# uncbiag/OAI_analysis_2

Hardware: NVIDIA B200
Metric: knee volumes/sec (seg+ICON reg+warp) (higher is better)
Workload: dtype fp16 operands / fp32 accumulate (tcgen05 kind::f16), the full-resolution decoder layers read fp16 hi+lo activations (dc2: skip input only; dc1); fp32 registration; fp64 warp coordinates

## Files before the change

### oai_analysis_2_b200/csrc/api_conv.cu

```cuda
#include "../../include/oai_b200.h"
#include "api_common.h"
#include "conv_api.h"
#include "conv_igemm.cuh"

#include <cuda_bf16.h>
#include <cuda_fp16.h>

#include <cstring>
#include <vector>

namespace oai {

cudaError_t conv_igemm_launch(const ConvIgemmParams& p, const CUtensorMap& tm0, const CUtensorMap& tm1, int num_sms,
                              cudaStream_t stream);
cudaError_t conv_overflow_count(unsigned int* count, bool reset, cudaStream_t stream);

namespace {

constexpr int kFlagForcePerTap = 1;
constexpr int kFlagBaseOffFormula = 2;
constexpr int kFlagForceKd1 = 4;
constexpr int kFlagNoFastPath = 8;
constexpr int kFlagWideN = 16;
constexpr int kFlagWideRows = 32;
// ... 20 lines not shown

int build_chunks(const ConvSpec& s, Plan* pl) {
  int n = 0;
  const int cs[2] = {s.c0, s.c1};
  for (int src = 0; src < 2; ++src) {
    const int c = cs[src];
    if (c == 0) continue;
    const bool spl = split_src(s.terms, src);
    const int wide = spl ? 2 * c : c;
    for (int j = 0; j * 64 < wide; ++j) {
      OAI_REQUIRE(n < kMaxChunks, "conv plan: more than %d K chunks", kMaxChunks);
      pl->chunks[n++] = Chunk{src, j * 64, s.terms == 3 ? 1 : 0, spl ? 1 : 0};
    }
    if (s.terms == 3)
      for (int j = 0; j * 64 < c; ++j) {
        OAI_REQUIRE(n < kMaxChunks, "conv plan: more than %d K chunks", kMaxChunks);
        pl->chunks[n++] = Chunk{src, j * 64, 2, 0};
      }
  }
  pl->nch = n;
  return 0;
}

int make_plan(const ConvSpec& s, Plan* pl, int d_cnt = 0) {
  const int D = s.D, H = s.H, W = s.W, c0 = s.c0, c1 = s.c1, cout = s.cout, pointwise = s.kind, flags = s.flags;
  OAI_REQUIRE(D > 0 && H > 0 && W > 0 && c0 > 0 && c1 >= 0 && cout > 0, "conv plan: bad dims");
  OAI_REQUIRE(c0 % 8 == 0 && c1 % 8 == 0, "conv plan: channel counts must be multiples of 8 (got %d,%d)", c0, c1);
  OAI_REQUIRE(s.terms >= 1 && s.terms <= 5,
              "conv plan: terms=%d (1 = 16-bit, 2 = split activations, 3 = split both, 4 / 5 = split the second / first "
              "source's activations only)", s.terms);
  OAI_REQUIRE((!split_src(s.terms, 0) || s.split0) && (!split_src(s.terms, 1) || c1 == 0 || s.split1),
              "conv plan: terms=%d needs the split sources stored as [hi | lo] planes", s.terms);
  OAI_REQUIRE(s.terms < 4 || c1 > 0, "conv plan: terms=%d is for two-source layers", s.terms);
  OAI_REQUIRE((!s.split0 || c0 % 32 == 0) && (!s.split1 || c1 % 64 == 0) && (c1 == 0 || c0 % 64 == 0),
              "conv plan: split / concatenated sources need 64-channel multiples (got %d,%d)", c0, c1);
  pl->TW = W < 128 ? W : 128;
  OAI_REQUIRE(128 % pl->TW == 0 && W % pl->TW == 0, "conv plan: W=%d must divide or be a multiple of 128", W);
  pl->TH = 128 / pl->TW;
  OAI_REQUIRE(H % pl->TH == 0, "conv plan: H=%d not a multiple of the %d-row M tile", H, pl->TH);
  const int ntile = (!pointwise && cout > 128 && !(flags & kFlagWideN)) ? 128 : 256;
  pl->nhalf = (cout + ntile - 1) / ntile;
  OAI_REQUIRE(cout % pl->nhalf == 0, "conv plan: cout=%d not divisible into %d N splits", cout, pl->nhalf);
  pl->cph = cout / pl->nhalf;
  OAI_REQUIRE(pl->cph % 32 == 0, "conv plan: cout per split (%d) must be a multiple of 32", pl->cph);
  OAI_REQUIRE(cout <= 512, "conv plan: cout=%d exceeds the 512-float bias staging area", cout);
  if (d_cnt <= 0) d_cnt = D;
  int R = 512 / pl->cph < 8 ? 512 / pl->cph : 8;
  if (R > d_cnt) R = d_cnt;
  pl->R = R;
  pl->Rd = R;
  pl->up_groups = 1;
  pl->pingpong = 0;
  if (build_chunks(s, pl)) return 1;
  const int c0v = split_src(s.terms, 0) ? 2 * c0 : c0;
  pl->k16 = (c1 == 0 && c0v <= 32) ? (c0v <= 16 ? 1 : 2) : 4;
  pl->row_bytes = (c1 == 0 && c0v == 32 && !(flags & kFlagWideRows)) ? 64 : 128;
  const int rb = pl->row_bytes;
  const int nch = pl->nch;
  if (pointwise == 2) {
    pl->mode = kModeUp2;
    pl->kd_per_block = 1;
    pl->R = 512 / pl->cph < 8 ? 512 / pl->cph : 8;
    if (pl->R >= 2 && !(flags & (kFlagNoFastPath | kFlagBaseOffFormula | kFlagNoPingPong))) {
      pl->R /= 2;
      pl->pingpong = 1;
    }
    pl->Rd = 1;
    pl->up_groups = 8 / pl->R;
    pl->wblock_bytes = pl->R * pl->cph * rb;
    pl->nblk = nch;
    pl->n_wbuf = 2;
  } else if (pointwise) {
    pl->mode = kModePointwise;
    pl->kd_per_block = 1;
    pl->wblock_bytes = pl->cph * rb;
    pl->nblk = nch;
    pl->n_wbuf = 3;
  } else if (pl->TW == 128 && pl->cph <= 64 && !(flags & kFlagForcePerTap)) {
    pl->mode = kModeRowShared;
    pl->kd_per_block = 3;
    pl->wblock_bytes = 9 * pl->cph * rb;
    pl->nblk = nch * 3;
    pl->n_wbuf = 2;
  } else {
    pl->mode = kModePerTap;
    pl->kd_per_block = (pl->cph <= 128 && !(flags & kFlagForceKd1)) ? 3 : 1;
    pl->wblock_bytes = pl->kd_per_block * pl->cph * rb;
    pl->nblk = nch * (pl->kd_per_block == 3 ? 9 : 27);
    pl->n_wbuf = pl->kd_per_block == 3 ? 2 : 3;
  }
  pl->nkh = 1;
  if (pl->mode == kModeRowShared && rb == 64 && nch == 1 &&
      !(flags & (kFlagOneKhRow | kFlagNoFastPath | kFlagBaseOffFormula))) {
    pl->nkh = 3;
    pl->n_wbuf = 1;
  }
  pl->astage_bytes = (pl->mode == kModeRowShared ? 130 : 128) * rb * pl->nkh;
  pl->astage_stride = (pl->astage_bytes + 1023u) & ~1023u;
  const size_t wstride = (static_cast<size_t>(pl->wblock_bytes) * pl->nkh + 1023u) & ~size_t(1023);
  pl->stationary = 0;
  if (pl->nkh == 3) pl->stationary = 1;
  if (pl->mode == kModeUp2 && pl->pingpong && pl->nblk <= 4 && pl->nblk * wstride + 4 * pl->astage_stride <= kSmemBudget) {
    pl->stationary = 1;
    pl->n_wbuf = pl->nblk;
  }
  const size_t left = kSmemBudget - pl->n_wbuf * wstride;
  int ns = static_cast<int>(left / pl->astage_stride);
  if (ns > 8) ns = 8;
  OAI_REQUIRE(ns >= 2, "conv plan: shared memory budget leaves %d A stages", ns);
  pl->n_astage = ns;
  return 0;
}

size_t plan_wpack_bytes(const Plan& pl) {
  return static_cast<size_t>(pl.nhalf) * pl.up_groups * pl.nblk * pl.wblock_bytes;
}

typedef CUresult (*EncodeTiledFn)(CUtensorMap*, CUtensorMapDataType, cuuint32_t, void*, const cuuint64_t*,
                                  const cuuint64_t*, const cuuint32_t*, const cuuint32_t*, CUtensorMapInterleave,
                                  CUtensorMapSwizzle, CUtensorMapL2promotion, CUtensorMapFloatOOBfill);
// ... 96 lines not shown
  if (s.terms == 3) { q[1].resize(nw); q[2].resize(nw); }
  for (size_t f = 0; f < static_cast<size_t>(cout) * cin; ++f) {
    double carry = 0.0;
    for (int t = 0; t < ktaps; ++t) {
      const double v = static_cast<double>(w[f * ktaps + t]) + (s.kind == 2 ? 0.0 : carry);
      const uint16_t h = to16(static_cast<float>(v), fmt);
      q[0][f * ktaps + t] = h;
      carry = v - static_cast<double>(from16(h, fmt));
      if (s.terms == 3) {
        const float wf = w[f * ktaps + t];
        const uint16_t hi = to16(wf, fmt);
        q[1][f * ktaps + t] = hi;
        q[2][f * ktaps + t] = to16(wf - from16(hi, fmt), fmt);
      }
    }
  }
  const int cs[2] = {s.c0, s.c1};
  const int ngroups = pl.up_groups;
  for (int nh = 0; nh < pl.nhalf; ++nh)
    for (int tg = 0; tg < ngroups; ++tg)
      for (int b = 0; b < pl.nblk; ++b) {
        uint8_t* blk = out + ((static_cast<size_t>(nh) * ngroups + tg) * pl.nblk + b) * pl.wblock_bytes;
        int c, kh = 0, kw0 = 0, nkw = 1, kdlo = 0, nkd = 1;
        if (pl.mode == kModeRowShared) {
          c = b / 3; kh = b % 3; nkw = 3; nkd = 3;
        } else if (pl.mode == kModePerTap && pl.kd_per_block == 3) {
          c = b / 9; const int r = b % 9; kh = r / 3; kw0 = r % 3; nkd = 3;
        } else if (pl.mode == kModePerTap) {
          c = b / 27; const int r = b % 27; kh = r / 9; kw0 = (r / 3) % 3; kdlo = r % 3;
        } else {
          c = b;
        }
        const Chunk& ck = pl.chunks[c];
        const int csrc = cs[ck.src], cbase = ck.src == 0 ? 0 : s.c0;
        const std::vector<uint16_t>& qq = q[ck.wsel];
        const int nstack = pl.mode == kModeUp2 ? pl.R : nkd;
        for (int kwi = 0; kwi < nkw; ++kwi)
          for (int ti = 0; ti < nstack; ++ti) {
            int tap;
            if (pl.mode == kModeUp2) tap = tg * pl.R + ti;
            else if (s.kind == 1) tap = 0;
            else tap = ((kdlo + nkd - 1 - ti) * 3 + kh) * 3 + kw0 + kwi;
            for (int co = 0; co < pl.cph; ++co) {
              const int r = (kwi * nstack + ti) * pl.cph + co;
              const uint16_t* wrow = qq.data() + (static_cast<size_t>(nh * pl.cph + co) * cin) * ktaps;
              for (int j = 0; j < 64 && j * 2 < pl.row_bytes; ++j) {
                const int v = ck.cc + j;
                if (v >= (ck.dup ? 2 * csrc : csrc)) break;
                const int ci = cbase + (ck.dup ? v % csrc : v);
                const uint16_t h = wrow[static_cast<size_t>(ci) * ktaps + tap];
                memcpy(blk + swz_off(r, j, pl.row_bytes), &h, 2);
              }
            }
          }
      }
  return 0;
}

int conv_run(const ConvSpec& s, const ConvLaunch& a, cudaStream_t st) {
  const int D = s.D, H = s.H, W = s.W, c0 = s.c0, c1 = s.c1, cout = s.cout;
  int d_lo = 0, d_cnt = D, h_lo = 0, h_cnt = H;
  if (a.region) {
    d_lo = a.region[0]; d_cnt = a.region[1]; h_lo = a.region[2]; h_cnt = a.region[3];
    OAI_REQUIRE(d_lo >= 0 && d_cnt >= 1 && d_lo + d_cnt <= D && h_lo >= 0 && h_cnt >= 1 && h_lo + h_cnt <= H,
                "conv: region [%d,+%d)x[%d,+%d) outside %dx%d", d_lo, d_cnt, h_lo, h_cnt, D, H);
  }
  Plan pl;
  if (make_plan(s, &pl, d_cnt)) return 1;
  const int hp_lo = h_lo / pl.TH;
  const int hp_cnt = (h_lo + h_cnt + pl.TH - 1) / pl.TH - hp_lo;
  const HeadFuse* head = a.head;
  OAI_REQUIRE(a.src0 && a.wpack && a.bias, "conv: null pointer");
  OAI_REQUIRE(!head || (pl.cph == 64 && pl.nhalf == 1), "conv head: the fused head needs a 64-channel layer");
  OAI_REQUIRE((c1 == 0) == (a.src1 == nullptr), "conv: src1/c1 mismatch");
  const size_t need = plan_wpack_bytes(pl);
  OAI_REQUIRE(a.wpack_bytes == need, "conv: packed weights are %zu bytes, geometry needs %zu", a.wpack_bytes, need);
  OAI_REQUIRE(a.obase % 16 == 0 && a.osN % 16 == 0 && a.osD % 16 == 0 && a.osH % 16 == 0 && a.osW % 16 == 0 &&
                  a.out_lo_off % 16 == 0 && (head || (reinterpret_cast<uintptr_t>(a.out) & 31) == 0),
              "conv: output base and strides must keep 32-byte alignment");
  OAI_REQUIRE(!(head && a.out_split), "conv head: the fused head writes class maps, not a split activation");

  ConvIgemmParams p;
  memset(&p, 0, sizeof(p));
  p.NT = a.NT; p.D = D; p.H = H; p.W = W;
  p.TW = pl.TW; p.TH = pl.TH; p.R = pl.R;
  p.cout = pl.cph; p.nhalf = pl.nhalf;
  p.nchunks = pl.nch; p.k16_steps = pl.k16; p.row_bytes = pl.row_bytes;
  for (int c = 0; c < pl.nch; ++c) {
    p.chunk_src[c] = static_cast<uint8_t>(pl.chunks[c].src);
    p.chunk_cc[c] = static_cast<uint16_t>(pl.chunks[c].cc);
  }
  p.mode = pl.mode; p.kd_per_block = pl.kd_per_block; p.nblk = pl.nblk / pl.nkh;
  p.wblock_bytes = pl.wblock_bytes * pl.nkh; p.n_wbuf = pl.n_wbuf; p.n_astage = pl.n_astage;
  p.nkh = pl.nkh;
  p.acc_pingpong = pl.pingpong;
  p.w_stationary = pl.stationary;
  p.astage_bytes = pl.astage_bytes; p.astage_stride = pl.astage_stride;
  p.ab_format = s.fmt; p.relu = a.relu;
  p.base_off_mode = (s.flags & kFlagBaseOffFormula) ? 1 : 0;
  p.no_fast_path = (s.flags & kFlagNoFastPath) ? 1 : 0;
  p.wpack = static_cast<const uint8_t*>(a.wpack);
  p.bias = a.bias;
  p.out = a.out;
  p.obase = a.obase; p.osN = a.osN; p.osD = a.osD; p.osH = a.osH; p.osW = a.osW;
  p.out_split = a.out_split; p.out_lo_off = a.out_lo_off;
  p.d_lo = d_lo; p.d_cnt = d_cnt; p.hp_lo = hp_lo; p.hp_cnt = hp_cnt;
  p.Rd = pl.Rd; p.up_groups = pl.up_groups;
  p.nunits = a.NT * ((d_cnt + pl.Rd - 1) / pl.Rd) * (hp_cnt * (W / pl.TW)) * pl.up_groups * pl.nhalf;
  if (pl.mode == kModeUp2) {
    const long long vox = a.osW / 2;
    for (int t = 0; t < 8; ++t)
      p.tap_off[t] = ((static_cast<long long>(t >> 2) * 2 * H + ((t >> 1) & 1)) * 2 * W + (t & 1)) * vox;
  }
  if (head) p.head = *head;

  OAI_REQUIRE(pl.mode != kModeUp2 || (c1 == 0 && !head), "conv: up2 mode takes one source and no fused head");
  const int bw = pl.mode == kModeRowShared ? 130 : pl.TW;
  const int bh = pl.TH * pl.nkh;
  CUtensorMap tm0, tm1;
  if (make_act_tmap(&tm0, a.src0, s.split0 ? 2 * c0 : c0, W, H, D, a.NT, bw, bh, s.fmt, pl.row_bytes)) return 1;
  if (a.src1) {
    if (make_act_tmap(&tm1, a.src1, s.split1 ? 2 * c1 : c1, W, H, D, a.NT, bw, bh, s.fmt)) return 1;
  } else {
    tm1 = tm0;
  }
  ProfEntry* pe = nullptr;
  if (g_prof_on) {
    if (g_prof_used == g_prof.size()) {
      ProfEntry ne;
      if (cudaEventCreate(&ne.a) != cudaSuccess || cudaEventCreate(&ne.b) != cudaSuccess)
        return fail("conv profile: cannot create events");
      g_prof.push_back(ne);
    }
    pe = &g_prof[g_prof_used++];
    const double taps = s.kind == 0 ? 27.0 : (s.kind == 1 ? 1.0 : 8.0);
    pe->flops = 2.0 * a.NT * D * H * W * static_cast<double>(cout) * (c0 + c1) * taps;
    pe->exec_flops = 2.0 * a.NT * static_cast<double>(d_cnt) * hp_cnt * pl.TH * W * static_cast<double>(cout) * taps *
                     (static_cast<double>(pl.nch) * pl.k16 * 16);
    prof_record(pe->a, st);
  }
  cudaError_t e = conv_igemm_launch(p, tm0, tm1, num_sms(), st);
  if (pe) prof_record(pe->b, st);
  g_launches.fetch_add(1, std::memory_order_relaxed);
  return check_cuda(e, "conv_igemm launch");
}

}

using namespace oai;

namespace {
ConvSpec spec_of(int D, int H, int W, int c0, int c1, int cout, int pointwise, int ab_format, int flags) {
  ConvSpec s;
  s.D = D; s.H = H; s.W = W; s.c0 = c0; s.c1 = c1; s.split0 = 0; s.split1 = 0; s.cout = cout; s.kind = pointwise;
  s.terms = 1; s.fmt = ab_format; s.flags = flags;
  return s;
}
}

extern "C" int oai_conv3d_igemm_plan(int D, int H, int W, int c0, int c1, int cout, int pointwise, int flags,
// ... 169 lines not shown
```

### oai_analysis_2_b200/csrc/conv_api.h

```cpp
#pragma once
#include <cstddef>
#include <cuda_runtime.h>

#include "conv_igemm.cuh"

namespace oai {

struct ConvSpec {
  int D, H, W;
  int c0, c1;
  int split0, split1;
  int cout;
  int kind;
  int terms;
  int fmt;
  int flags;
};

struct ConvLaunch {
  const void* src0;
  const void* src1;
  int NT;
  const void* wpack;
  size_t wpack_bytes;
  const float* bias;
  int relu;
  void* out;
  long long obase, osN, osD, osH, osW;
  int out_split;
  long long out_lo_off;
  const int* region;
  const HeadFuse* head;
};

size_t conv_wpack_bytes(const ConvSpec& s);
int conv_pack_weights(const ConvSpec& s, const float* w, void* dst, size_t dst_bytes);
int conv_run(const ConvSpec& s, const ConvLaunch& a, cudaStream_t st);

inline HeadFuse make_head_fuse(int ncls, const float* head_w, const float* head_b, float* out, const int* vol_dims,
                               const int* geom, int tile0, const int* crop_zyx, int out_mode) {
  HeadFuse hd;
  hd.enabled = 1; hd.ncls = ncls; hd.out_mode = out_mode; hd.w = head_w; hd.b = head_b; hd.out = out;
  hd.VD = vol_dims[0]; hd.VH = vol_dims[1]; hd.VW = vol_dims[2];
  hd.ed = geom[3]; hd.eh = geom[4]; hd.ew = geom[5];
  hd.od = geom[6]; hd.oh = geom[7]; hd.ow = geom[8];
  hd.gh = geom[10]; hd.gw = geom[11]; hd.tile0 = tile0;
  hd.cz = crop_zyx[0]; hd.cy = crop_zyx[1]; hd.cx = crop_zyx[2];
  return hd;
}

}
```

### oai_analysis_2_b200/csrc/conv_igemm.cu

```cuda
#include "conv_igemm.cuh"
#include "ptx.cuh"

#include <cuda_bf16.h>
#include <cuda_fp16.h>

namespace oai {

namespace {

constexpr int kThreads = 384;
constexpr int kEpiGroups = 2;
constexpr int kTmemCols = 512;

__device__ unsigned int g_fp16_overflow = 0;

struct BlockInfo {
  int c, kh, kw, kdlo, nkd;
  int ns;
};

__device__ __forceinline__ BlockInfo decode_block(const ConvIgemmParams& p, int b) {
  BlockInfo bi;
  if (p.mode == kModeRowShared) {
    bi.c = p.nkh == 3 ? b : b / 3;
    bi.kh = p.nkh == 3 ? 0 : b % 3;
    bi.kw = 0;
    bi.kdlo = 0;
    bi.nkd = 3;
  } else if (p.mode == kModePerTap) {
    if (p.kd_per_block == 3) {
      bi.c = b / 9;
      const int r = b % 9;
      bi.kh = r / 3;
      bi.kw = r % 3;
      bi.kdlo = 0;
      bi.nkd = 3;
    } else {
      bi.c = b / 27;
      const int r = b % 27;
      bi.kh = r / 9;
      bi.kw = (r / 3) % 3;
      bi.kdlo = r % 3;
      bi.nkd = 1;
    }
  } else {
    bi.c = b;
    bi.kh = 1;
    bi.kw = 1;
    bi.kdlo = 1;
    bi.nkd = 1;
  }
  bi.ns = (p.mode == kModeUp2) ? p.R : bi.nkd;
  return bi;
}

struct UnitInfo {
  int n, d0, h0, w0, nh;
  int tg;
  int rd;
  int ra;
};

__device__ __forceinline__ UnitInfo decode_unit(const ConvIgemmParams& p, int u) {
  UnitInfo ui;
  const int npw = p.W / p.TW;
  const int np = npw * p.hp_cnt, ndg = (p.d_cnt + p.Rd - 1) / p.Rd;
  if (p.w_stationary) {
    const int per_key = np * ndg * p.NT;
    const int key = u / per_key;
    u -= key * per_key;
    ui.tg = key % p.up_groups;
    ui.nh = key / p.up_groups;
  } else {
    ui.nh = u % p.nhalf;
    u /= p.nhalf;
    ui.tg = u % p.up_groups;
    u /= p.up_groups;
  }
  const int patch = u % np;
  u /= np;
  ui.d0 = p.d_lo + (u % ndg) * p.Rd;
  ui.n = u / ndg;
  ui.h0 = (p.hp_lo + patch / npw) * p.TH;
  ui.w0 = (patch % npw) * p.TW;
  ui.rd = min(p.Rd, p.d_lo + p.d_cnt - ui.d0);
  ui.ra = (p.mode == kModeUp2) ? p.R : ui.rd;
  return ui;
}

template <int FMT>
__device__ __forceinline__ uint32_t pack2(float a, float b) {
  if (FMT == 0) {
    __half2 h = __floats2half2_rn(a, b);
    return *reinterpret_cast<uint32_t*>(&h);
  }
  __nv_bfloat162 h = __floats2bfloat162_rn(a, b);
  return *reinterpret_cast<uint32_t*>(&h);
}

__device__ __forceinline__ void st_global_256(void* p, const uint32_t* v) {
  asm volatile("st.global.v8.b32 [%0], {%1,%2,%3,%4,%5,%6,%7,%8};" ::"l"(p), "r"(v[0]), "r"(v[1]), "r"(v[2]), "r"(v[3]),
               "r"(v[4]), "r"(v[5]), "r"(v[6]), "r"(v[7])
               : "memory");
}

template <int FMT>
__device__ __forceinline__ uint32_t pack2_residual(float a, float b, uint32_t hi) {
// ... 107 lines not shown
    const int ag = acc0 + g0;
    const int keep = min(max(f0 - ag, 0), ng);
    const uint32_t bl = b_lo + static_cast<uint32_t>(g0) * c.tap16;
    if (keep > 0)
      umma_f16_ss_lohi(tmem_base + static_cast<uint32_t>(ag) * c.cout, a_lo, bl, c.desc_hi32,
                       c.idesc_1 + static_cast<uint32_t>(keep - 1) * c.idesc_step, 1u);
    if (keep < ng)
      umma_f16_ss_lohi(tmem_base + static_cast<uint32_t>(ag + keep) * c.cout, a_lo,
                       bl + static_cast<uint32_t>(keep) * c.tap16, c.desc_hi32,
                       c.idesc_1 + static_cast<uint32_t>(ng - keep - 1) * c.idesc_step, 0u);
  }
}

template <int NKW, int K16N, int PER, int NKH>
__device__ __forceinline__ void mma_issuer_fast(const ConvIgemmParams& p, const uint32_t tmem_base0, uint8_t* abuf,
                                                uint8_t* wbuf, const uint32_t wstride, uint64_t* full_a,
                                                uint64_t* empty_a, uint64_t* full_w, uint64_t* empty_w,
                                                uint64_t* acc_full0, uint64_t* acc_empty0) {
  const int mode = p.mode, R_acc = p.R, nblk = p.nblk, nst = p.n_astage, nwb = p.n_wbuf, Dm1 = p.D - 1;
  const uint32_t rowb = static_cast<uint32_t>(p.row_bytes), sbo = 8u * rowb, lay = rowb == 128u ? 2u : 4u;
  IssueConsts c;
  c.cout = static_cast<uint32_t>(p.cout);
  c.tap16 = (c.cout * rowb) >> 4;
  c.kw_step = rowb >> 4;
  c.desc_hi32 = (sbo >> 4) | (1u << 14) | (lay << 29);
  c.idesc_1 = umma_idesc_f16(128, c.cout, p.ab_format);
  c.idesc_step = (c.cout >> 3) << 17;
  const uint32_t a_lo0 = ((smem_u32(abuf) & 0x3FFFF) >> 4) | (1u << 16), a_step = p.astage_stride >> 4;
  const uint32_t w_lo0 = ((smem_u32(wbuf) & 0x3FFFF) >> 4) | (1u << 16), w_step = wstride >> 4;
  const bool up2 = mode == kModeUp2;
  const bool one_kd = mode == kModePointwise || up2;
  const bool kd_cycle = mode == kModePerTap && p.kd_per_block == 1;
  const int ns = up2 ? R_acc : ((one_kd || kd_cycle) ? 1 : 3);
  const int a_inc = up2 ? 0 : 1;
  c.b_kw = static_cast<uint32_t>(ns) * c.tap16;
  c.kh_a = (130u * rowb) >> 4;
  c.kh_b = 3u * c.b_kw;
  const bool stationary = p.w_stationary != 0;
  int prev_key = -1;
  const bool leader = elect_one();
  int stage = 0, wb = 0;
  uint32_t aphase = 0, wphase = 0;
  uint32_t ub0 = 0, ub1 = 0;
  uint32_t a_lo = a_lo0;
  int half = 0;
  for (int u = blockIdx.x; u < p.nunits; u += gridDim.x) {
    const UnitInfo ui = decode_unit(p, u);
// ... 62 lines not shown
      }
      if (release && leader) umma_commit(&empty_w[wb]);
      if (++wb == nwb) {
        wb = 0;
        if (reload) wphase ^= 1u;
      }
    }
    if (leader && signaled != all_acc) {
      for (int a = 0; a < ra; ++a)
        if (!((signaled >> a) & 1u)) umma_commit(&acc_full[a]);
    }
    if (this_half) ub1 = use_bits ^ all_acc;
    else ub0 = use_bits ^ all_acc;
  }
  __syncwarp();
}

__device__ __forceinline__ void mma_issuer_general(const ConvIgemmParams& p, const uint32_t tmem_base, uint8_t* abuf,
                                                   uint8_t* wbuf, const uint32_t wstride, uint64_t* full_a,
                                                   uint64_t* empty_a, uint64_t* full_w, uint64_t* empty_w,
                                                   uint64_t* acc_full, uint64_t* acc_empty) {
  const int mode = p.mode, R_acc = p.R, cout = p.cout, nblk = p.nblk, nst = p.n_astage, nwb = p.n_wbuf, Dm1 = p.D - 1,
            kpb = p.kd_per_block;
  const int nkw = (mode == kModeRowShared) ? 3 : 1;
  const int k16n = p.k16_steps;
  const uint32_t rowb = static_cast<uint32_t>(p.row_bytes), sbo = 8u * rowb, lay = rowb == 128u ? 2u : 4u;
  const uint32_t cout128 = static_cast<uint32_t>(cout) * rowb;
  const bool up2 = mode == kModeUp2;
  const bool leader = elect_one();
  int stage = 0, wb = 0;
  uint32_t aphase = 0, wphase = 0, use_bits = 0;
  for (int u = blockIdx.x; u < p.nunits; u += gridDim.x) {
    const UnitInfo ui = decode_unit(p, u);
    const int d0 = ui.d0, ra = ui.ra, rd = ui.rd;
    const uint32_t all_acc = (1u << ra) - 1u;
    uint32_t touched = 0, signaled = 0;
    int kd_it = 0;
    for (int b = 0; b < nblk; ++b) {
      int kdlo = 0, nkd = 3;
      if (mode == kModePointwise || up2) { kdlo = 1; nkd = 1; }
      else if (mode == kModePerTap && kpb == 1) { kdlo = kd_it; nkd = 1; kd_it = kd_it == 2 ? 0 : kd_it + 1; }
      const int ns = up2 ? R_acc : nkd;
      const int kdhi = kdlo + nkd - 1;
      const int dlo = max(0, d0 + kdlo - 1);
      const int dhi = min(Dm1, d0 + rd - 1 + kdhi - 1);
      const bool last_blk = b == nblk - 1;
      mbar_wait(&full_w[wb], wphase, 300 + wb);
      int a_first = up2 ? 0 : dlo - kdhi + 1 - d0;
      for (int dp = dlo; dp <= dhi; ++dp, a_first += (up2 ? 0 : 1)) {
        mbar_wait(&full_a[stage], aphase, 400 + stage);
        tc_fence_after();
        const int acc0 = max(a_first, 0);
        const int ti_lo = acc0 - a_first;
        const int nt = min(ns - 1, ra - 1 - a_first) - ti_lo + 1;
        const uint32_t a_base = smem_u32(abuf + static_cast<size_t>(stage) * p.astage_stride);
        const uint32_t w_base = smem_u32(wbuf + static_cast<size_t>(wb) * wstride);
        const int ti_hi = ti_lo + nt - 1;
        for (int kw = 0; kw < nkw; ++kw) {
          int ti = ti_lo;
          while (ti <= ti_hi) {
            const int a0 = a_first + ti;
            const uint32_t f = (touched >> a0) & 1u;
            int len = 1;
            while (ti + len <= ti_hi && ((touched >> (a0 + len)) & 1u) == f && (len + 1) * cout <= 256) ++len;
            if (!f) {
              for (int j = 0; j < len; ++j)
                mbar_wait(&acc_empty[a0 + j], ((use_bits >> (a0 + j)) & 1u) ^ 1u, 500 + a0 + j);
              tc_fence_after();
            }
            const uint32_t idesc = umma_idesc_f16(128, static_cast<uint32_t>(len * cout), p.ab_format);
            const uint32_t a_addr = a_base + static_cast<uint32_t>(kw) * rowb;
            const uint32_t b_addr = w_base + static_cast<uint32_t>(kw * ns + ti) * cout128;
            const uint32_t boff = p.base_off_mode ? ((a_addr >> 7) & 7u) : 0u;
            const uint32_t d_addr = tmem_base + static_cast<uint32_t>(a0 * cout);
            if (leader) {
              for (int k16 = 0; k16 < k16n; ++k16) {
                const uint64_t adesc = umma_desc_kmajor(a_addr + k16 * 32, sbo, boff, lay);
                const uint64_t bdesc = umma_desc_kmajor(b_addr + k16 * 32, sbo, 0, lay);
                umma_f16_ss(d_addr, adesc, bdesc, idesc, (f | (k16 > 0)) ? 1u : 0u);
              }
            }
            touched |= ((1u << len) - 1u) << a0;
            ti += len;
          }
        }
        const bool publish = last_blk && a_first >= 0 && a_first < ra;
        if (leader) {
          umma_commit(&empty_a[stage]);
          if (publish) umma_commit(&acc_full[a_first]);
        }
        if (publish) signaled |= 1u << a_first;
        if (++stage == nst) {
          stage = 0;
          aphase ^= 1u;
// ... 98 lines not shown
    if (lane == 0) {
      int wb = 0, prev_key = -1;
      uint32_t phase = 0;
      for (int u = blockIdx.x; u < p.nunits; u += gridDim.x) {
        const UnitInfo ui = decode_unit(p, u);
        const uint8_t* src = p.wpack + static_cast<size_t>(ui.nh * p.up_groups + ui.tg) * p.nblk * p.wblock_bytes;
        const int key = ui.nh * p.up_groups + ui.tg;
        if (p.w_stationary && key == prev_key) continue;
        prev_key = key;
        for (int b = 0; b < p.nblk; ++b) {
          mbar_wait(&empty_w[wb], phase ^ 1u, 200 + wb);
          mbar_arrive_expect_tx(&full_w[wb], p.wblock_bytes);
          bulk_load(wbuf + static_cast<size_t>(wb) * wstride, src + static_cast<size_t>(b) * p.wblock_bytes,
                    p.wblock_bytes, &full_w[wb]);
          if (++wb == p.n_wbuf) {
            wb = 0;
            phase ^= 1u;
          }
        }
      }
    }
  } else if (warp == 2) {
    const bool general = p.base_off_mode || p.no_fast_path;
    const int nkw_rt = (p.mode == kModeRowShared) ? 3 : 1;
    const int per_rt = max(1, 256 / p.cout);
#define OAI_ISSUE(NKW, K16N, PER) \
  mma_issuer_fast<NKW, K16N, PER, 1>(p, tmem_base, abuf, wbuf, wstride, full_a, empty_a, full_w, empty_w, acc_full, acc_empty)
#define OAI_ISSUE_GENERAL() \
  mma_issuer_general(p, tmem_base, abuf, wbuf, wstride, full_a, empty_a, full_w, empty_w, acc_full, acc_empty)
    if (general) OAI_ISSUE_GENERAL();
    else if (nkw_rt == 3 && p.k16_steps == 4 && per_rt == 4) OAI_ISSUE(3, 4, 4);
    else if (nkw_rt == 3 && p.k16_steps == 2 && per_rt == 4 && p.nkh == 3)
      mma_issuer_fast<3, 2, 4, 3>(p, tmem_base, abuf, wbuf, wstride, full_a, empty_a, full_w, empty_w, acc_full, acc_empty);
    else if (nkw_rt == 3 && p.k16_steps == 2 && per_rt == 4) OAI_ISSUE(3, 2, 4);
    else if (nkw_rt == 1 && p.k16_steps == 4 && per_rt == 4) OAI_ISSUE(1, 4, 4);
    else if (nkw_rt == 1 && p.k16_steps == 4 && per_rt == 2) OAI_ISSUE(1, 4, 2);
    else if (nkw_rt == 1 && p.k16_steps == 4 && per_rt == 1) OAI_ISSUE(1, 4, 1);
    else OAI_ISSUE_GENERAL();
#undef OAI_ISSUE_GENERAL
#undef OAI_ISSUE
  } else if (warp >= 4) {
    const int q = warp & 3;
    const int eg = (warp - 4) >> 2;
    const int epi_variant = (p.ab_format ? 4 : 0) + (p.out_split ? 2 : 0) + (p.relu ? 1 : 0);
    const uint32_t s_bias_addr = smem_u32(s_bias), s_head_addr = smem_u32(s_head);
    const int m = q * 32 + lane;
    const int th = m / p.TW, tw = m % p.TW;
// ... 139 lines not shown
```

### oai_analysis_2_b200/csrc/conv_igemm.cuh

```cuda
#pragma once
#include <cstdint>
#include <cuda.h>
#include <cuda_runtime.h>

namespace oai {

constexpr int kMaxChunks = 48;

enum ConvMode : int {
  kModeRowShared = 0,
  kModePerTap = 1,
  kModePointwise = 2,
  kModeUp2 = 3,
};

struct HeadFuse {
  int enabled;
  int ncls, out_mode;
  const float* w;
  const float* b;
  float* out;
  int VD, VH, VW;
  int ed, eh, ew, od, oh, ow, gh, gw, tile0;
  int cz, cy, cx;
};

struct ConvIgemmParams {
  int NT, D, H, W;
  int TW, TH;
  int R;
  int Rd;
  int up_groups;
  long long tap_off[8];
  int d_lo, d_cnt;
  int hp_lo, hp_cnt;
  int cout;
  int nhalf;
  int nchunks;
  uint16_t chunk_cc[kMaxChunks];
  uint8_t chunk_src[kMaxChunks];
  int k16_steps;
  int row_bytes;
  int mode;
  int kd_per_block;
  int nblk;
  uint32_t wblock_bytes;
  int n_wbuf;
  int nkh;
  int w_stationary;
  int acc_pingpong;
  int n_astage;
  uint32_t astage_bytes;
  uint32_t astage_stride;
  int ab_format;
  int relu;
  int no_fast_path;
  int base_off_mode;
  const uint8_t* wpack;
// ... 11 lines not shown
```

### oai_analysis_2_b200/csrc/seg_net.cu

```cuda
#include "../../include/oai_b200.h"
#include "api_common.h"
#include "conv_api.h"
#include "seg_misc.cuh"

#include <nvtx3/nvToolsExt.h>

#include <algorithm>
#include <cmath>
#include <cstring>
#include <map>
#include <set>
#include <string>
#include <vector>

using namespace oai;

namespace {

struct LayerDef {
  const char* name;
  char kind;
  int cin, cout;
  int level;
  int c_first;
};

const LayerDef kLayers[] = {
    {"ec0", 'c', 1, 32, 0, 0},     {"ec1", 'c', 32, 64, 0, 0},    {"ec2", 'c', 64, 64, 1, 0},
    {"ec3", 'c', 64, 128, 1, 0},   {"ec4", 'c', 128, 128, 2, 0},  {"ec5", 'c', 128, 256, 2, 0},
    {"ec6", 'c', 256, 256, 3, 0},  {"ec7", 'c', 256, 512, 3, 0},  {"dc9", 'u', 512, 512, 3, 0},
    {"dc8", 't', 768, 256, 2, 512}, {"dc7", 't', 256, 256, 2, 0}, {"dc6", 'u', 256, 256, 2, 0},
// ... 106 lines not shown
  for (int a = 0; a < 3; ++a) { n0.lo[a] = overlap[a]; n0.hi[a] = tile[a] - overlap[a] - 1; }
  n0 = clampbox(n0, 0);
  region[DC1] = n0;
  region[DC2] = dil(n0, 1, 0);
  Box need = dil(n0, 2, 0);
  const int ups[2][3] = {{DC3, DC4, DC5}, {DC6, DC7, DC8}};
  for (int i = 0; i < 2; ++i) {
    const int lvl = i + 1;
    const Box q = half(need, lvl);
    region[ups[i][0]] = q;
    region[ups[i][1]] = q;
    region[ups[i][2]] = dil(q, 1, lvl);
    need = dil(q, 2, lvl);
  }
  region[DC9] = half(need, 3);
}

struct NamedTensor {
  const float* data;
  std::vector<long long> shape;
  long long numel;
};

int device_copy(const void* host, size_t bytes, void** dev) {
  if (int rc = check_cuda(cudaMalloc(dev, bytes), "seg_create: cudaMalloc")) return rc;
  return check_cuda(cudaMemcpy(*dev, host, bytes, cudaMemcpyHostToDevice), "seg_create: cudaMemcpy");
}

}

extern "C" int oai_seg_needed_regions(const int* tile_zyx, const int* overlap_zyx, int* boxes) {
  OAI_REQUIRE(tile_zyx && overlap_zyx && boxes, "seg_needed_regions: null pointer");
  Box region[kNumLayers];
  needed_regions(tile_zyx, overlap_zyx, region);
  for (int l = 0; l < kNumLayers; ++l)
    for (int a = 0; a < 3; ++a) {
      boxes[l * 6 + a] = region[l].lo[a];
      boxes[l * 6 + 3 + a] = region[l].hi[a];
    }
  return 0;
}

extern "C" int oai_seg_layer_terms(int precision, int* terms17) {
  OAI_REQUIRE(terms17 != nullptr, "seg_layer_terms: null pointer");
  OAI_REQUIRE(precision >= OAI_SEG_PRECISION_FP16 && precision <= OAI_SEG_PRECISION_FP16X3,
              "seg_layer_terms: unknown precision %d", precision);
// ... 38 lines not shown
                h->tile[a]);
    OAI_REQUIRE(h->overlap[a] >= 0 && 2 * h->overlap[a] < h->tile[a],
                "seg_create: overlap_size must be smaller than half the patch size");
  }
  if (cfg->precision == OAI_SEG_PRECISION_CUSTOM) {
    for (int l = 0; l < kNumLayers; ++l) {
      h->terms[l] = l == 0 ? 1 : cfg->layer_terms[l];
      OAI_REQUIRE(h->terms[l] >= 1 && h->terms[l] <= 5 && (h->terms[l] < 4 || kLayers[l].c_first > 0),
                  "seg_create: layer_terms[%d]=%d", l, h->terms[l]);
    }
  } else if (oai_seg_layer_terms(cfg->precision, h->terms)) {
    return 1;
  }
  for (int t = 0; t < kNumTensors; ++t) {
    const int c = kTensors[t].consumers[0];
    const bool is_skip = t == T_SYN0 || t == T_SYN1 || t == T_SYN2;
    const int tm = c >= 0 ? h->terms[c] : 1;
    h->split[t] = tm == 2 || tm == 3 || (tm == 4 && is_skip) || (tm == 5 && !is_skip);
  }
  for (int i = 0; i < 3; ++i)
    if (h->split[kPoolOf[i][1]]) h->split[kPoolOf[i][0]] = 1;
  needed_regions(h->tile, h->overlap, h->region);
  h->has_region = h->overlap[0] || h->overlap[1] || h->overlap[2];

  std::set<std::string> consumed;
  auto take = [&](const std::string& key, std::initializer_list<long long> shape, const NamedTensor** out) -> int {
    auto it = sd.find(key);
    OAI_REQUIRE(it != sd.end(), "seg_create: missing key %s in state_dict", key.c_str());
    const NamedTensor& t = it->second;
    bool ok = t.shape.size() == shape.size() && t.data != nullptr;
    size_t i = 0;
    for (long long s : shape) ok = ok && t.shape[i++] == s;
    OAI_REQUIRE(ok, "seg_create: size mismatch for %s", key.c_str());
    *out = &t;
    consumed.insert(key);
    return 0;
  };
  const int ncls = cfg->n_classes;
  for (int l = 0; l < kNumLayers; ++l) {
    const LayerDef& L = kLayers[l];
    const std::string nm = L.name;
    const int k = L.kind == 'u' ? 2 : 3, taps = k * k * k, ci = L.cin, co = L.cout;
    const NamedTensor *w, *b = nullptr, *g = nullptr, *beta = nullptr, *mean = nullptr, *var = nullptr;
    if (L.kind == 'c') {
      if (take(nm + ".0.weight", {co, ci, k, k, k}, &w)) return 1;
    } else {
// ... 18 lines not shown
        for (int t = 0; t < taps; ++t) {
          const size_t src = L.kind == 'c' ? (static_cast<size_t>(o) * ci + i) * taps + t
                                           : (static_cast<size_t>(i) * co + o) * taps + (L.kind == 't' ? taps - 1 - t : t);
          wf[(static_cast<size_t>(o) * ci + i) * taps + t] = static_cast<float>(static_cast<double>(w->data[src]) * s);
        }
    }
    PackedLayer& P = h->layers[l];
    if (device_copy(bf.data(), bf.size() * sizeof(float), reinterpret_cast<void**>(&P.bias))) return 1;
    if (l == EC0) {
      std::vector<float> w27(27 * co);
      for (int t = 0; t < 27; ++t)
        for (int o = 0; o < co; ++o) w27[t * co + o] = wf[static_cast<size_t>(o) * 27 + t];
      if (device_copy(w27.data(), w27.size() * sizeof(float), reinterpret_cast<void**>(&h->stem_w))) return 1;
      continue;
    }
    ConvSpec& s = P.spec;
    s.D = dims_at(h, L.level, 0); s.H = dims_at(h, L.level, 1); s.W = dims_at(h, L.level, 2);
    s.c0 = L.c_first ? L.c_first : ci;
    s.c1 = ci - s.c0;
    s.cout = co;
    s.kind = L.kind == 'u' ? 2 : 0;
    s.terms = h->terms[l];
    s.fmt = cfg->ab_format;
    s.flags = 0;
    s.split0 = s.split1 = 0;
    ConvSpec ps = s;
    ps.split0 = s.terms == 2 || s.terms == 3 || s.terms == 5;
    ps.split1 = (s.terms == 2 || s.terms == 3 || s.terms == 4) && s.c1 > 0;
    P.w_bytes = conv_wpack_bytes(ps);
    OAI_REQUIRE(P.w_bytes > 0, "seg_create: layer %s: %s", L.name, oai_last_error());
    std::vector<uint8_t> img(P.w_bytes);
    if (conv_pack_weights(ps, wf.data(), img.data(), img.size())) return 1;
    if (device_copy(img.data(), img.size(), &P.w)) return 1;
  }
  {
    const NamedTensor *w0, *b0 = nullptr;
    if (take("dc0.weight", {ncls, 64, 1, 1, 1}, &w0)) return 1;
    if (cfg->bias && take("dc0.bias", {ncls}, &b0)) return 1;
    std::vector<float> hb(ncls, 0.f);
    if (b0) std::copy(b0->data, b0->data + ncls, hb.begin());
    if (device_copy(w0->data, static_cast<size_t>(ncls) * 64 * sizeof(float), reinterpret_cast<void**>(&h->head_w)) ||
        device_copy(hb.data(), ncls * sizeof(float), reinterpret_cast<void**>(&h->head_b)))
      return 1;
  }
  for (const auto& kv : sd)
    OAI_REQUIRE(consumed.count(kv.first), "seg_create: unexpected key %s in state_dict", kv.first.c_str());
  guard.h = nullptr;
// ... 35 lines not shown
  OAI_REQUIRE(out_mode >= 0 && out_mode <= 2, "seg_forward: out_mode=%d", out_mode);
  OAI_REQUIRE((reinterpret_cast<uintptr_t>(workspace) & 255) == 0, "seg_forward: workspace must be 256-byte aligned");
  cudaStream_t st = static_cast<cudaStream_t>(stream);
  int eff[3], grid[3];
  tiling(h, vol_dims, eff, grid);
  for (int a = 0; a < 3; ++a) {
    const int padded = eff[a] * grid[a] + 2 * h->overlap[a] - vol_dims[a];
    OAI_REQUIRE(vol_dims[a] >= 1 && !(vol_dims[a] < 2 && padded > 0),
                "seg_forward: reflect padding needs at least 2 samples along a padded axis");
  }
  const int T = grid[0] * grid[1] * grid[2];
  const int nb = tiles_per_batch <= 0 ? T : std::min(T, tiles_per_batch);
  size_t offs[kNumTensors];
  const size_t need = plan_workspace(h, nb, offs);
  OAI_REQUIRE(workspace_bytes >= need, "seg_forward: workspace holds %zu bytes, %d tiles per batch need %zu",
              workspace_bytes, nb, need);
  uint8_t* ws = static_cast<uint8_t*>(workspace);
  auto buf = [&](int t) { return static_cast<void*>(ws + offs[t]); };
  const int geom[12] = {h->tile[0], h->tile[1], h->tile[2], eff[0], eff[1], eff[2],
                        h->overlap[0], h->overlap[1], h->overlap[2], grid[0], grid[1], grid[2]};
  const int crop_zyx[3] = {h->cfg.overlap_xyz[2], h->cfg.overlap_xyz[0], h->cfg.overlap_xyz[1]};
  const int fmt = h->cfg.ab_format;

  auto conv = [&](int l, int NT, int t0, int t1, int tout) -> int {
    const LayerDef& L = kLayers[l];
    const PackedLayer& P = h->layers[l];
    ConvSpec s = P.spec;
    s.split0 = h->split[t0];
    s.split1 = t1 >= 0 ? h->split[t1] : 0;
    ConvLaunch a;
    a.src0 = buf(t0);
    a.src1 = t1 >= 0 ? buf(t1) : nullptr;
    a.NT = NT; a.wpack = P.w; a.wpack_bytes = P.w_bytes; a.bias = P.bias; a.relu = 1;
    a.out = buf(tout);
    a.obase = 0;
    a.out_split = h->split[tout];
    a.out_lo_off = L.cout;
    const long long cp = (a.out_split ? 2ll : 1ll) * L.cout;
    if (L.kind == 'u') {
      a.osN = 8ll * s.D * s.H * s.W * cp; a.osD = 8ll * s.H * s.W * cp; a.osH = 4ll * s.W * cp; a.osW = 2 * cp;
    } else {
      a.osN = 1ll * s.D * s.H * s.W * cp; a.osD = 1ll * s.H * s.W * cp; a.osH = 1ll * s.W * cp; a.osW = cp;
    }
    int region[4];
    a.region = nullptr;
    if (h->has_region && l >= DC9) {
      const Box& b = h->region[l];
      region[0] = b.lo[0]; region[1] = b.hi[0] - b.lo[0] + 1; region[2] = b.lo[1]; region[3] = b.hi[1] - b.lo[1] + 1;
      a.region = region;
    }
    a.head = nullptr;
    return conv_run(s, a, st);
  };
  auto pool = [&](int i, int NT) -> int {
    const int tin = kPoolOf[i][0], tout = kPoolOf[i][1];
    const TensorDef& d = kTensors[tin];
    return maxpool2_launch(buf(tin), buf(tout), NT, dims_at(h, d.level, 0), dims_at(h, d.level, 1),
                           dims_at(h, d.level, 2), d.channels, h->split[tin], h->split[tout], fmt, st);
  };

  nvtxRangePushA("oai.seg_forward");
  int rc = 0;
  for (int t0 = 0; t0 < T && !rc; t0 += nb) {
    const int NT = std::min(nb, T - t0);
    StemParams sp;
    sp.vol = vol; sp.VD = vol_dims[0]; sp.VH = vol_dims[1]; sp.VW = vol_dims[2];
    sp.td = geom[0]; sp.th = geom[1]; sp.tw = geom[2];
    sp.ed = geom[3]; sp.eh = geom[4]; sp.ew = geom[5];
    sp.od = geom[6]; sp.oh = geom[7]; sp.ow = geom[8];
    sp.gh = geom[10]; sp.gw = geom[11];
    sp.tile0 = t0; sp.ntiles = NT; sp.c0 = 32; sp.w = h->stem_w; sp.b = h->layers[EC0].bias; sp.out = buf(T_E0);
    sp.fmt = fmt; sp.out_split = h->split[T_E0];
    rc = stem_launch(sp, st)
         || conv(EC1, NT, T_E0, -1, T_SYN0)
// ... 4 lines not shown
         || conv(EC4, NT, T_P1, -1, T_E4)
         || conv(EC5, NT, T_E4, -1, T_SYN2)
         || pool(2, NT)
         || conv(EC6, NT, T_P2, -1, T_E6)
         || conv(EC7, NT, T_E6, -1, T_E7)
         || conv(DC9, NT, T_E7, -1, T_D9)
         || conv(DC8, NT, T_D9, T_SYN2, T_D8)
         || conv(DC7, NT, T_D8, -1, T_D7)
         || conv(DC6, NT, T_D7, -1, T_D6)
         || conv(DC5, NT, T_D6, T_SYN1, T_D5)
         || conv(DC4, NT, T_D5, -1, T_D4)
         || conv(DC3, NT, T_D4, -1, T_D3)
         || conv(DC2, NT, T_D3, T_SYN0, T_D2);
    if (rc) break;
    const PackedLayer& P = h->layers[DC1];
    ConvSpec s = P.spec;
    s.split0 = h->split[T_D2];
    HeadFuse hd = make_head_fuse(h->cfg.n_classes, h->head_w, h->head_b, out, vol_dims, geom, t0, crop_zyx, out_mode);
    const int region[4] = {geom[6], geom[3], geom[7], geom[4]};
    ConvLaunch a;
    a.src0 = buf(T_D2); a.src1 = nullptr; a.NT = NT; a.wpack = P.w; a.wpack_bytes = P.w_bytes; a.bias = P.bias;
    a.relu = 1; a.out = nullptr; a.obase = a.osN = a.osD = a.osH = a.osW = 0; a.out_split = 0; a.out_lo_off = 0;
    a.region = region; a.head = &hd;
    rc = conv_run(s, a, st);
  }
  nvtxRangePop();
  return rc;
}
```

Before: 9.633.

## Add kh-shared conv mode to skip W-halo work in full-res decoder layers

Adds a conv mode where the A tile is a narrower TW×(TH+2) box and the three kh taps share one staged tile, with kw split across weight blocks. This allows the DC2 and DC1 layers to compute only the W range needed for the cropped output instead of the full tile width, removing the overlap-halo columns. The W range is split into a 32-aligned main launch plus a small remainder launch, and tile sizes are chosen to minimise the tile count. This adds extra launches and narrower tiles, which may reduce MMA efficiency, and the path can be disabled with an environment variable.

New measurement: 10.28, median of 6. +6.8%, better.

```diff
diff --git a/oai_analysis_2_b200/csrc/api_conv.cu b/oai_analysis_2_b200/csrc/api_conv.cu
--- a/oai_analysis_2_b200/csrc/api_conv.cu
+++ b/oai_analysis_2_b200/csrc/api_conv.cu
@@ -66,7 +66,7 @@
   return 0;
 }
 
-int make_plan(const ConvSpec& s, Plan* pl, int d_cnt = 0) {
+int make_plan(const ConvSpec& s, Plan* pl, int d_cnt = 0, int tw = 32) {
   const int D = s.D, H = s.H, W = s.W, c0 = s.c0, c1 = s.c1, cout = s.cout, pointwise = s.kind, flags = s.flags;
   OAI_REQUIRE(D > 0 && H > 0 && W > 0 && c0 > 0 && c1 >= 0 && cout > 0, "conv plan: bad dims");
   OAI_REQUIRE(c0 % 8 == 0 && c1 % 8 == 0, "conv plan: channel counts must be multiples of 8 (got %d,%d)", c0, c1);
@@ -79,9 +79,11 @@
   OAI_REQUIRE((!s.split0 || c0 % 32 == 0) && (!s.split1 || c1 % 64 == 0) && (c1 == 0 || c0 % 64 == 0),
               "conv plan: split / concatenated sources need 64-channel multiples (got %d,%d)", c0, c1);
   pl->TW = W < 128 ? W : 128;
-  OAI_REQUIRE(128 % pl->TW == 0 && W % pl->TW == 0, "conv plan: W=%d must divide or be a multiple of 128", W);
   pl->TH = 128 / pl->TW;
-  OAI_REQUIRE(H % pl->TH == 0, "conv plan: H=%d not a multiple of the %d-row M tile", H, pl->TH);
+  if (!(flags & kConvFlagKhShared)) {
+    OAI_REQUIRE(128 % pl->TW == 0 && W % pl->TW == 0, "conv plan: W=%d must divide or be a multiple of 128", W);
+    OAI_REQUIRE(H % pl->TH == 0, "conv plan: H=%d not a multiple of the %d-row M tile", H, pl->TH);
+  }
   const int ntile = (!pointwise && cout > 128 && !(flags & kFlagWideN)) ? 128 : 256;
   pl->nhalf = (cout + ntile - 1) / ntile;
   OAI_REQUIRE(cout % pl->nhalf == 0, "conv plan: cout=%d not divisible into %d N splits", cout, pl->nhalf);
@@ -120,6 +122,17 @@
     pl->wblock_bytes = pl->cph * rb;
     pl->nblk = nch;
     pl->n_wbuf = 3;
+  } else if (flags & kConvFlagKhShared) {
+    OAI_REQUIRE(pl->cph <= 64 && rb == 128 && (tw == 8 || tw == 16 || tw == 32) && W >= tw && H >= 128 / tw,
+                "conv plan: kh-shared mode needs cout <= 64, 64-channel chunks and a grid of at least one %d-wide tile "
+                "(cout=%d, %dx%d)", tw, cout, H, W);
+    pl->mode = kModeKhShared;
+    pl->kd_per_block = 3;
+    pl->wblock_bytes = 9 * pl->cph * rb;
+    pl->nblk = nch * 3;
+    pl->n_wbuf = 2;
+    pl->TW = tw;
+    pl->TH = 128 / tw;
   } else if (pl->TW == 128 && pl->cph <= 64 && !(flags & kFlagForcePerTap)) {
     pl->mode = kModeRowShared;
     pl->kd_per_block = 3;
@@ -139,7 +152,7 @@
     pl->nkh = 3;
     pl->n_wbuf = 1;
   }
-  pl->astage_bytes = (pl->mode == kModeRowShared ? 130 : 128) * rb * pl->nkh;
+  pl->astage_bytes = (pl->mode == kModeRowShared ? 130 : pl->mode == kModeKhShared ? 128 + 2 * pl->TW : 128) * rb * pl->nkh;
   pl->astage_stride = (pl->astage_bytes + 1023u) & ~1023u;
   const size_t wstride = (static_cast<size_t>(pl->wblock_bytes) * pl->nkh + 1023u) & ~size_t(1023);
   pl->stationary = 0;
@@ -282,8 +295,11 @@
       for (int b = 0; b < pl.nblk; ++b) {
         uint8_t* blk = out + ((static_cast<size_t>(nh) * ngroups + tg) * pl.nblk + b) * pl.wblock_bytes;
         int c, kh = 0, kw0 = 0, nkw = 1, kdlo = 0, nkd = 1;
+        const bool kh_inner = pl.mode == kModeKhShared;
         if (pl.mode == kModeRowShared) {
           c = b / 3; kh = b % 3; nkw = 3; nkd = 3;
+        } else if (kh_inner) {
+          c = b / 3; kw0 = b % 3; nkw = 3; nkd = 3;
         } else if (pl.mode == kModePerTap && pl.kd_per_block == 3) {
           c = b / 9; const int r = b % 9; kh = r / 3; kw0 = r % 3; nkd = 3;
         } else if (pl.mode == kModePerTap) {
@@ -300,6 +316,7 @@
             int tap;
             if (pl.mode == kModeUp2) tap = tg * pl.R + ti;
             else if (s.kind == 1) tap = 0;
+            else if (kh_inner) tap = ((kdlo + nkd - 1 - ti) * 3 + kh + kwi) * 3 + kw0;
             else tap = ((kdlo + nkd - 1 - ti) * 3 + kh) * 3 + kw0 + kwi;
             for (int co = 0; co < pl.cph; ++co) {
               const int r = (kwi * nstack + ti) * pl.cph + co;
@@ -319,16 +336,33 @@
 
 int conv_run(const ConvSpec& s, const ConvLaunch& a, cudaStream_t st) {
   const int D = s.D, H = s.H, W = s.W, c0 = s.c0, c1 = s.c1, cout = s.cout;
-  int d_lo = 0, d_cnt = D, h_lo = 0, h_cnt = H;
+  const bool kh_shared = (s.flags & kConvFlagKhShared) != 0;
+  int d_lo = 0, d_cnt = D, h_lo = 0, h_cnt = H, w_lo = 0, w_cnt = W;
   if (a.region) {
     d_lo = a.region[0]; d_cnt = a.region[1]; h_lo = a.region[2]; h_cnt = a.region[3];
     OAI_REQUIRE(d_lo >= 0 && d_cnt >= 1 && d_lo + d_cnt <= D && h_lo >= 0 && h_cnt >= 1 && h_lo + h_cnt <= H,
                 "conv: region [%d,+%d)x[%d,+%d) outside %dx%d", d_lo, d_cnt, h_lo, h_cnt, D, H);
   }
+  if (a.w_cnt) {
+    w_lo = a.w_lo; w_cnt = a.w_cnt;
+    OAI_REQUIRE(kh_shared, "conv: a w range needs a layer packed for kh-shared mode");
+    OAI_REQUIRE(w_lo >= 0 && w_cnt >= 1 && w_lo + w_cnt <= W, "conv: w range [%d,+%d) outside W=%d", w_lo, w_cnt, W);
+  }
+  int tw = 32, ntile = 0;
+  if (kh_shared)
+    for (int t = 32; t >= 8; t /= 2) {
+      if (t > W || 128 / t > H) continue;
+      const int n = ((w_cnt + t - 1) / t) * ((h_cnt + 128 / t - 1) / (128 / t));
+      if (ntile == 0 || n < ntile) { ntile = n; tw = t; }
+    }
   Plan pl;
-  if (make_plan(s, &pl, d_cnt)) return 1;
-  const int hp_lo = h_lo / pl.TH;
-  const int hp_cnt = (h_lo + h_cnt + pl.TH - 1) / pl.TH - hp_lo;
+  if (make_plan(s, &pl, d_cnt, tw)) return 1;
+  int tile_h_lo = h_lo, nph = (h_cnt + pl.TH - 1) / pl.TH, npw = (w_cnt + pl.TW - 1) / pl.TW;
+  if (!kh_shared) {
+    tile_h_lo = h_lo / pl.TH * pl.TH;
+    nph = (h_lo + h_cnt + pl.TH - 1) / pl.TH - h_lo / pl.TH;
+    npw = W / pl.TW;
+  }
   const HeadFuse* head = a.head;
   OAI_REQUIRE(a.src0 && a.wpack && a.bias, "conv: null pointer");
   OAI_REQUIRE(!head || (pl.cph == 64 && pl.nhalf == 1), "conv head: the fused head needs a 64-channel layer");
@@ -364,9 +398,9 @@
   p.out = a.out;
   p.obase = a.obase; p.osN = a.osN; p.osD = a.osD; p.osH = a.osH; p.osW = a.osW;
   p.out_split = a.out_split; p.out_lo_off = a.out_lo_off;
-  p.d_lo = d_lo; p.d_cnt = d_cnt; p.hp_lo = hp_lo; p.hp_cnt = hp_cnt;
+  p.d_lo = d_lo; p.d_cnt = d_cnt; p.h_lo = tile_h_lo; p.nph = nph; p.w_lo = kh_shared ? w_lo : 0; p.npw = npw;
   p.Rd = pl.Rd; p.up_groups = pl.up_groups;
-  p.nunits = a.NT * ((d_cnt + pl.Rd - 1) / pl.Rd) * (hp_cnt * (W / pl.TW)) * pl.up_groups * pl.nhalf;
+  p.nunits = a.NT * ((d_cnt + pl.Rd - 1) / pl.Rd) * (nph * npw) * pl.up_groups * pl.nhalf;
   if (pl.mode == kModeUp2) {
     const long long vox = a.osW / 2;
     for (int t = 0; t < 8; ++t)
@@ -376,7 +410,7 @@
 
   OAI_REQUIRE(pl.mode != kModeUp2 || (c1 == 0 && !head), "conv: up2 mode takes one source and no fused head");
   const int bw = pl.mode == kModeRowShared ? 130 : pl.TW;
-  const int bh = pl.TH * pl.nkh;
+  const int bh = pl.mode == kModeKhShared ? pl.TH + 2 : pl.TH * pl.nkh;
   CUtensorMap tm0, tm1;
   if (make_act_tmap(&tm0, a.src0, s.split0 ? 2 * c0 : c0, W, H, D, a.NT, bw, bh, s.fmt, pl.row_bytes)) return 1;
   if (a.src1) {
@@ -394,8 +428,8 @@
     }
     pe = &g_prof[g_prof_used++];
     const double taps = s.kind == 0 ? 27.0 : (s.kind == 1 ? 1.0 : 8.0);
-    pe->flops = 2.0 * a.NT * D * H * W * static_cast<double>(cout) * (c0 + c1) * taps;
-    pe->exec_flops = 2.0 * a.NT * static_cast<double>(d_cnt) * hp_cnt * pl.TH * W * static_cast<double>(cout) * taps *
+    pe->flops = 2.0 * a.NT * D * H * W * static_cast<double>(cout) * (c0 + c1) * taps * a.flop_share;
+    pe->exec_flops = 2.0 * a.NT * static_cast<double>(d_cnt) * nph * npw * 128 * static_cast<double>(cout) * taps *
                      (static_cast<double>(pl.nch) * pl.k16 * 16);
     prof_record(pe->a, st);
   }
diff --git a/oai_analysis_2_b200/csrc/conv_api.h b/oai_analysis_2_b200/csrc/conv_api.h
--- a/oai_analysis_2_b200/csrc/conv_api.h
+++ b/oai_analysis_2_b200/csrc/conv_api.h
@@ -5,6 +5,8 @@
 #include "conv_igemm.cuh"
 
 namespace oai {
+
+constexpr int kConvFlagKhShared = 256;
 
 struct ConvSpec {
   int D, H, W;
@@ -30,6 +32,8 @@
   int out_split;
   long long out_lo_off;
   const int* region;
+  int w_lo = 0, w_cnt = 0;
+  double flop_share = 1.0;
   const HeadFuse* head;
 };
 
diff --git a/oai_analysis_2_b200/csrc/conv_igemm.cu b/oai_analysis_2_b200/csrc/conv_igemm.cu
--- a/oai_analysis_2_b200/csrc/conv_igemm.cu
+++ b/oai_analysis_2_b200/csrc/conv_igemm.cu
@@ -25,6 +25,12 @@
     bi.c = p.nkh == 3 ? b : b / 3;
     bi.kh = p.nkh == 3 ? 0 : b % 3;
     bi.kw = 0;
+    bi.kdlo = 0;
+    bi.nkd = 3;
+  } else if (p.mode == kModeKhShared) {
+    bi.c = b / 3;
+    bi.kh = 0;
+    bi.kw = b % 3;
     bi.kdlo = 0;
     bi.nkd = 3;
   } else if (p.mode == kModePerTap) {
@@ -63,8 +69,8 @@
 
 __device__ __forceinline__ UnitInfo decode_unit(const ConvIgemmParams& p, int u) {
   UnitInfo ui;
-  const int npw = p.W / p.TW;
-  const int np = npw * p.hp_cnt, ndg = (p.d_cnt + p.Rd - 1) / p.Rd;
+  const int npw = p.npw;
+  const int np = npw * p.nph, ndg = (p.d_cnt + p.Rd - 1) / p.Rd;
   if (p.w_stationary) {
     const int per_key = np * ndg * p.NT;
     const int key = u / per_key;
@@ -81,8 +87,8 @@
   u /= np;
   ui.d0 = p.d_lo + (u % ndg) * p.Rd;
   ui.n = u / ndg;
-  ui.h0 = (p.hp_lo + patch / npw) * p.TH;
-  ui.w0 = (patch % npw) * p.TW;
+  ui.h0 = min(p.h_lo + (patch / npw) * p.TH, p.H - p.TH);
+  ui.w0 = min(p.w_lo + (patch % npw) * p.TW, p.W - p.TW);
   ui.rd = min(p.Rd, p.d_lo + p.d_cnt - ui.d0);
   ui.ra = (p.mode == kModeUp2) ? p.R : ui.rd;
   return ui;
@@ -236,7 +242,7 @@
   IssueConsts c;
   c.cout = static_cast<uint32_t>(p.cout);
   c.tap16 = (c.cout * rowb) >> 4;
-  c.kw_step = rowb >> 4;
+  c.kw_step = (mode == kModeKhShared ? static_cast<uint32_t>(p.TW) * rowb : rowb) >> 4;
   c.desc_hi32 = (sbo >> 4) | (1u << 14) | (lay << 29);
   c.idesc_1 = umma_idesc_f16(128, c.cout, p.ab_format);
   c.idesc_step = (c.cout >> 3) << 17;
@@ -345,7 +351,8 @@
                                                    uint64_t* acc_full, uint64_t* acc_empty) {
   const int mode = p.mode, R_acc = p.R, cout = p.cout, nblk = p.nblk, nst = p.n_astage, nwb = p.n_wbuf, Dm1 = p.D - 1,
             kpb = p.kd_per_block;
-  const int nkw = (mode == kModeRowShared) ? 3 : 1;
+  const int nkw = (mode == kModeRowShared || mode == kModeKhShared) ? 3 : 1;
+  const uint32_t a_tap = mode == kModeKhShared ? static_cast<uint32_t>(p.TW) * p.row_bytes : p.row_bytes;
   const int k16n = p.k16_steps;
   const uint32_t rowb = static_cast<uint32_t>(p.row_bytes), sbo = 8u * rowb, lay = rowb == 128u ? 2u : 4u;
   const uint32_t cout128 = static_cast<uint32_t>(cout) * rowb;
@@ -392,7 +399,7 @@
               tc_fence_after();
             }
             const uint32_t idesc = umma_idesc_f16(128, static_cast<uint32_t>(len * cout), p.ab_format);
-            const uint32_t a_addr = a_base + static_cast<uint32_t>(kw) * rowb;
+            const uint32_t a_addr = a_base + static_cast<uint32_t>(kw) * a_tap;
             const uint32_t b_addr = w_base + static_cast<uint32_t>(kw * ns + ti) * cout128;
             const uint32_t boff = p.base_off_mode ? ((a_addr >> 7) & 7u) : 0u;
             const uint32_t d_addr = tmem_base + static_cast<uint32_t>(a0 * cout);
@@ -537,7 +544,7 @@
     }
   } else if (warp == 2) {
     const bool general = p.base_off_mode || p.no_fast_path;
-    const int nkw_rt = (p.mode == kModeRowShared) ? 3 : 1;
+    const int nkw_rt = (p.mode == kModeRowShared || p.mode == kModeKhShared) ? 3 : 1;
     const int per_rt = max(1, 256 / p.cout);
 #define OAI_ISSUE(NKW, K16N, PER) \
   mma_issuer_fast<NKW, K16N, PER, 1>(p, tmem_base, abuf, wbuf, wstride, full_a, empty_a, full_w, empty_w, acc_full, acc_empty)
diff --git a/oai_analysis_2_b200/csrc/conv_igemm.cuh b/oai_analysis_2_b200/csrc/conv_igemm.cuh
--- a/oai_analysis_2_b200/csrc/conv_igemm.cuh
+++ b/oai_analysis_2_b200/csrc/conv_igemm.cuh
@@ -12,6 +12,7 @@
   kModePerTap = 1,
   kModePointwise = 2,
   kModeUp2 = 3,
+  kModeKhShared = 4,
 };
 
 struct HeadFuse {
@@ -33,7 +34,8 @@
   int up_groups;
   long long tap_off[8];
   int d_lo, d_cnt;
-  int hp_lo, hp_cnt;
+  int h_lo, nph;
+  int w_lo, npw;
   int cout;
   int nhalf;
   int nchunks;
diff --git a/oai_analysis_2_b200/csrc/seg_net.cu b/oai_analysis_2_b200/csrc/seg_net.cu
--- a/oai_analysis_2_b200/csrc/seg_net.cu
+++ b/oai_analysis_2_b200/csrc/seg_net.cu
@@ -7,6 +7,7 @@
 
 #include <algorithm>
 #include <cmath>
+#include <cstdlib>
 #include <cstring>
 #include <map>
 #include <set>
@@ -159,6 +160,11 @@
   long long numel;
 };
 
+bool w_halo_skip_disabled() {
+  const char* e = getenv("OAI_B200_SEG_W_HALO");
+  return e && e[0] == '0';
+}
+
 int device_copy(const void* host, size_t bytes, void** dev) {
   if (int rc = check_cuda(cudaMalloc(dev, bytes), "seg_create: cudaMalloc")) return rc;
   return check_cuda(cudaMemcpy(*dev, host, bytes, cudaMemcpyHostToDevice), "seg_create: cudaMemcpy");
@@ -243,6 +249,7 @@
     if (h->split[kPoolOf[i][1]]) h->split[kPoolOf[i][0]] = 1;
   needed_regions(h->tile, h->overlap, h->region);
   h->has_region = h->overlap[0] || h->overlap[1] || h->overlap[2];
+  const bool skip_w_halo = h->has_region && !w_halo_skip_disabled();
 
   std::set<std::string> consumed;
   auto take = [&](const std::string& key, std::initializer_list<long long> shape, const NamedTensor** out) -> int {
@@ -307,7 +314,7 @@
     s.kind = L.kind == 'u' ? 2 : 0;
     s.terms = h->terms[l];
     s.fmt = cfg->ab_format;
-    s.flags = 0;
+    s.flags = (skip_w_halo && (l == DC2 || l == DC1) && s.W % 128 == 0) ? kConvFlagKhShared : 0;
     s.split0 = s.split1 = 0;
     ConvSpec ps = s;
     ps.split0 = s.terms == 2 || s.terms == 3 || s.terms == 5;
@@ -389,6 +396,18 @@
   const int crop_zyx[3] = {h->cfg.overlap_xyz[2], h->cfg.overlap_xyz[0], h->cfg.overlap_xyz[1]};
   const int fmt = h->cfg.ab_format;
 
+  auto conv_w_box = [&](const ConvSpec& s, ConvLaunch a, int w_lo, int w_hi) -> int {
+    const int w_cnt = w_hi - w_lo + 1, main = w_cnt / 32 * 32, rest = w_cnt - main;
+    if (main) {
+      a.w_lo = w_lo; a.w_cnt = main; a.flop_share = static_cast<double>(main) / w_cnt;
+      if (int rc = conv_run(s, a, st)) return rc;
+    }
+    if (!rest) return 0;
+    a.w_cnt = std::min((rest + 7) / 8 * 8, w_cnt);
+    a.w_lo = w_hi + 1 - a.w_cnt;
+    a.flop_share = static_cast<double>(rest) / w_cnt;
+    return conv_run(s, a, st);
+  };
   auto conv = [&](int l, int NT, int t0, int t1, int tout) -> int {
     const LayerDef& L = kLayers[l];
     const PackedLayer& P = h->layers[l];
@@ -417,6 +436,7 @@
       a.region = region;
     }
     a.head = nullptr;
+    if (a.region && (s.flags & kConvFlagKhShared)) return conv_w_box(s, a, h->region[l].lo[2], h->region[l].hi[2]);
     return conv_run(s, a, st);
   };
   auto pool = [&](int i, int NT) -> int {
@@ -467,7 +487,7 @@
     a.src0 = buf(T_D2); a.src1 = nullptr; a.NT = NT; a.wpack = P.w; a.wpack_bytes = P.w_bytes; a.bias = P.bias;
     a.relu = 1; a.out = nullptr; a.obase = a.osN = a.osD = a.osH = a.osW = 0; a.out_split = 0; a.out_lo_off = 0;
     a.region = region; a.head = &hd;
-    rc = conv_run(s, a, st);
+    rc = (s.flags & kConvFlagKhShared) ? conv_w_box(s, a, geom[8], geom[8] + geom[5] - 1) : conv_run(s, a, st);
   }
   nvtxRangePop();
   return rc;
```
